# jskvrna/MonoSOWA

Hardware: AMD Instinct MI355X
Metric: MonoDETR training img/s (KITTI 1280x384) (higher is better)
Workload: dtype f32; 1 GPU; MonoDETR resnet50 KITTI 1280x384, fwd+criterion+bwd+AdamW step, per-GPU batch 16, synthetic images + random pseudo-labels; global_batch=16, per_gpu_batch=16, parallelism=dp1, accumulation_micro_steps=1, mixed_cameras=False, queries=550, tuned=True

## Files before the change

include/monosowa_attn.h:

```cpp
#ifndef MONOSOWA_ATTN_H
#define MONOSOWA_ATTN_H
#ifdef __cplusplus
extern "C" {
#endif

#define MONO_ATTN_E_NULLPTR (-1)
#define MONO_ATTN_E_SHAPE (-2)

typedef struct { long long batch, head, token; } mono_attn_strides;

int mono_attn_forward_f32(const float *q, const float *k, const float *v, float *o, float *lse, int B, int H, int Lq,
                          int Lk, int head_dim, mono_attn_strides sq, mono_attn_strides sk, mono_attn_strides sv,
                          mono_attn_strides so, float softmax_scale, float dropout_p, unsigned long long seed,
                          void *stream);

int mono_attn_backward_f32(const float *q, const float *k, const float *v, const float *o, const float *lse,
                           const float *dout, float *dq, float *dk, float *dv, float *delta, int B, int H, int Lq,
                           int Lk, int head_dim, mono_attn_strides sq, mono_attn_strides sk, mono_attn_strides sv,
                           mono_attn_strides so, mono_attn_strides sdq, mono_attn_strides sdk, mono_attn_strides sdv,
                           float softmax_scale, float dropout_p, unsigned long long seed, void *stream);

int mono_attn_forward_masked_f32(const float *q, const float *k, const float *v, const unsigned char *key_padding_mask, float *o,
                                 float *lse, int B, int H, int Lq, int Lk, int head_dim, mono_attn_strides sq,
                                 mono_attn_strides sk, mono_attn_strides sv, mono_attn_strides so, float softmax_scale,
                                 float dropout_p, unsigned long long seed, void *stream);
int mono_attn_backward_masked_f32(const float *q, const float *k, const float *v, const unsigned char *key_padding_mask,
                                  const float *o, const float *lse, const float *dout, float *dq, float *dk, float *dv, float *delta,
                                  int B, int H, int Lq, int Lk, int head_dim, mono_attn_strides sq, mono_attn_strides sk,
                                  mono_attn_strides sv, mono_attn_strides so, mono_attn_strides sdq, mono_attn_strides sdk,
                                  mono_attn_strides sdv, float softmax_scale, float dropout_p, unsigned long long seed,
                                  void *stream);

long long mono_attn_keep_words(int B, int H, int Lq, int Lk);
int mono_attn_forward_keep_f32(const float *q, const float *k, const float *v, const unsigned char *key_padding_mask,
                               unsigned *keep_bits, float *o, float *lse, int B, int H, int Lq, int Lk, int head_dim,
                               mono_attn_strides sq, mono_attn_strides sk, mono_attn_strides sv, mono_attn_strides so,
                               float softmax_scale, float dropout_p, unsigned long long seed, void *stream);
int mono_attn_backward_keep_f32(const float *q, const float *k, const float *v, const unsigned char *key_padding_mask,
                                const unsigned *keep_bits, const float *o, const float *lse, const float *dout, float *dq, float *dk,
                                float *dv, float *delta, int B, int H, int Lq, int Lk, int head_dim, mono_attn_strides sq,
                                mono_attn_strides sk, mono_attn_strides sv, mono_attn_strides so, mono_attn_strides sdq,
                                mono_attn_strides sdk, mono_attn_strides sdv, float softmax_scale, float dropout_p,
                                unsigned long long seed, void *stream);

#ifdef __cplusplus
}
#endif
#endif
```

monosowa_amd/csrc/flash_attn.hip:

```cpp
#include <hip/hip_runtime.h>

#include "../../include/monosowa_attn.h"

namespace attn {

typedef float f32x16 __attribute__((ext_vector_type(16)));

#ifndef ATTN_FWD_WAVES
#define ATTN_FWD_WAVES 4
#endif
#ifndef ATTN_BWD_WAVES
#define ATTN_BWD_WAVES 3
#endif
#ifndef ATTN_PREFETCH
#define ATTN_PREFETCH 0
#endif
#ifndef ATTN_OPDEPTH
#define ATTN_OPDEPTH 0
#endif
#ifndef ATTN_OPDEPTH_KV
#define ATTN_OPDEPTH_KV 0
#endif
#ifndef ATTN_EARLY_STORE
#define ATTN_EARLY_STORE 0
#endif
#ifndef ATTN_PRIO
#define ATTN_PRIO 0
#endif
#define ATTN_PRIO_MFMA()  do { if (ATTN_PRIO == 1) __builtin_amdgcn_s_setprio(2); else if (ATTN_PRIO == 2) __builtin_amdgcn_s_setprio(0); } while (0)
#define ATTN_PRIO_VALU()  do { if (ATTN_PRIO == 1) __builtin_amdgcn_s_setprio(0); else if (ATTN_PRIO == 2) __builtin_amdgcn_s_setprio(2); } while (0)
#ifndef ATTN_SKIP
#define ATTN_SKIP 0
#endif
constexpr int kBlockQ = 128;
constexpr int kTileK = 64;
constexpr int kKStride = 36;
constexpr int kVStride = 40;

struct Strides { long long b, h, t; };

struct Args {
  const float *q, *k, *v;
  float *o, *lse;
  const float *dout, *delta;
  float *dq, *dk, *dv;
  int H, Lq, Lk;
  Strides sq, sk, sv, so;
  Strides sdq, sdk, sdv;
  float scale_log2;
  float scale;
  unsigned drop_thr16;
  float drop_scale;
  unsigned seed_lo, seed_hi;
  const unsigned char *kmask;
  unsigned *keep;
};
__device__ __forceinline__ long long keep_index(const Args &a, int bh, int q_block, int k_tile, int slot) {
  const int n_qb = (a.Lq + 127) >> 7, n_kt = (a.Lk + 63) >> 6;
  return (((long long)bh * n_qb + q_block) * n_kt + k_tile) * 256 + slot;
}

__device__ __forceinline__ unsigned mix32(unsigned x) {
  x ^= x >> 16; x *= 0x85EBCA6Bu; x ^= x >> 13; x *= 0xC2B2AE35u; x ^= x >> 16;
  return x;
}
__device__ __forceinline__ unsigned drop_bits(unsigned head_seed, unsigned q, unsigned kp) {
  if (ATTN_SKIP & 32) return head_seed + q * 0x9E3779B1u + kp * 0x85EBCA77u;
  return mix32(head_seed + q * 0x9E3779B1u + kp * 0x85EBCA77u);
}
__device__ __forceinline__ unsigned head_seed_of(const Args &a, unsigned bh) {
  return mix32(a.seed_lo ^ (bh * 0xC2B2AE3Du)) ^ a.seed_hi;
}
__device__ __forceinline__ float4 ld4(const float *p) { return *reinterpret_cast<const float4 *>(p); }
__device__ __forceinline__ float xhalf(float v) { return __shfl_xor(v, 32); }
__device__ __forceinline__ f32x16 mfma(float a, float b, f32x16 c) { return __builtin_amdgcn_mfma_f32_32x32x2f32(a, b, c, 0, 0, 0); }

template <bool DROP, bool MASK, bool BITS>
constexpr int fwd_waves() { return (DROP && (MASK || !BITS)) ? 3 : ATTN_FWD_WAVES; }
template <bool DROP, bool MASK = false, bool BITS = false>
__global__ __launch_bounds__(256, (fwd_waves<DROP, MASK, BITS>())) void fwd_kernel(const Args a) {
  __shared__ float Ks[2][kTileK * kKStride];
  __shared__ float Vs[2][kTileK * kVStride];
  __shared__ unsigned long long Ms[2];
  const int lane = threadIdx.x & 63, wave = threadIdx.x >> 6, r = lane & 31, h = lane >> 5;
  const int bh = blockIdx.y, b = bh / a.H, hd = bh % a.H;
  const int q = blockIdx.x * kBlockQ + wave * 32 + r;
  const int qc = min(q, a.Lq - 1);
  const float *qp = a.q + b * a.sq.b + hd * a.sq.h + (long long)qc * a.sq.t + 16 * h;
  float qreg[16];
#pragma unroll
  for (int i = 0; i < 4; ++i) {
    const float4 t = ld4(qp + 4 * i);
    qreg[4 * i] = t.x * a.scale_log2; qreg[4 * i + 1] = t.y * a.scale_log2;
    qreg[4 * i + 2] = t.z * a.scale_log2; qreg[4 * i + 3] = t.w * a.scale_log2;
  }
  const float *kb = a.k + b * a.sk.b + hd * a.sk.h, *vb = a.v + b * a.sv.b + hd * a.sv.h;
  const int n_tiles = (a.Lk + kTileK - 1) / kTileK;
  float4 kr[2], vr[2];
  unsigned long long pad_next = 0;
  auto load_tile = [&](int kt) {
#pragma unroll
    for (int j = 0; j < 2; ++j) {
      const int idx = threadIdx.x + 256 * j, key = kt * kTileK + (idx >> 3), c = (idx & 7) * 4;
      const bool ok = key < a.Lk;
      kr[j] = ok ? ld4(kb + (long long)key * a.sk.t + c) : make_float4(0.f, 0.f, 0.f, 0.f);
      vr[j] = ok ? ld4(vb + (long long)key * a.sv.t + c) : make_float4(0.f, 0.f, 0.f, 0.f);
    }
    if (MASK && wave == 0) {
      const int key = kt * kTileK + lane;
      pad_next = __ballot(!(key < a.Lk && a.kmask[(long long)b * a.Lk + key] == 0));
    }
  };
  auto store_tile = [&](int buf) {
#pragma unroll
    for (int j = 0; j < 2; ++j) {
      const int idx = threadIdx.x + 256 * j, row = idx >> 3, c = (idx & 7) * 4;
      *reinterpret_cast<float4 *>(&Ks[buf][row * kKStride + c]) = kr[j];
      *reinterpret_cast<float4 *>(&Vs[buf][row * kVStride + c]) = vr[j];
    }
    if (MASK && threadIdx.x == 0) Ms[buf] = pad_next;
  };
  load_tile(0);
  store_tile(0);
  __syncthreads();

  const unsigned hseed = DROP ? head_seed_of(a, (unsigned)bh) : 0u;
  f32x16 o = {0.f, 0.f, 0.f, 0.f, 0.f, 0.f, 0.f, 0.f, 0.f, 0.f, 0.f, 0.f, 0.f, 0.f, 0.f, 0.f};
  float m = -INFINITY, lsum = 0.f;
  for (int kt = 0; kt < n_tiles; ++kt) {
    const int buf = kt & 1;
    if (kt + 1 < n_tiles) load_tile(kt + 1);
    f32x16 s0 = {0.f, 0.f, 0.f, 0.f, 0.f, 0.f, 0.f, 0.f, 0.f, 0.f, 0.f, 0.f, 0.f, 0.f, 0.f, 0.f}, s1 = s0;
    const float *k0 = &Ks[buf][r * kKStride + 16 * h], *k1 = k0 + 32 * kKStride;
    ATTN_PRIO_MFMA();
#pragma unroll
    for (int i = 0; i < 4; ++i) {
      const float4 a0 = ld4(k0 + 4 * i), a1 = ld4(k1 + 4 * i);
      s0 = mfma(a0.x, qreg[4 * i], s0);     s1 = mfma(a1.x, qreg[4 * i], s1);
      s0 = mfma(a0.y, qreg[4 * i + 1], s0); s1 = mfma(a1.y, qreg[4 * i + 1], s1);
      s0 = mfma(a0.z, qreg[4 * i + 2], s0); s1 = mfma(a1.z, qreg[4 * i + 2], s1);
      s0 = mfma(a0.w, qreg[4 * i + 3], s0); s1 = mfma(a1.w, qreg[4 * i + 3], s1);
    }
    ATTN_PRIO_VALU();
    const int key0 = kt * kTileK + 4 * h;
    if (MASK) {
      const unsigned long long tm = Ms[buf];
      const unsigned lo = __builtin_amdgcn_readfirstlane((unsigned)tm), hi = __builtin_amdgcn_readfirstlane((unsigned)(tm >> 32));
      const unsigned w0 = lo >> (4 * h), w1 = hi >> (4 * h);
#pragma unroll
      for (int v = 0; v < 16; ++v) {
        const int bit = 8 * (v >> 2) + (v & 3);
        if ((w0 >> bit) & 1u) s0[v] = -INFINITY;
        if ((w1 >> bit) & 1u) s1[v] = -INFINITY;
      }
    } else if (kt == n_tiles - 1 && (a.Lk & (kTileK - 1))) {
#pragma unroll
      for (int v = 0; v < 16; ++v) {
        const int key = key0 + 8 * (v >> 2) + (v & 3);
// ... 155 lines not shown
      for (int i = 0; i < 4; ++i) {
#if ATTN_PREFETCH
        const float4 ka = ka4[i], va = va4[i];
#else
        const float4 ka = (ATTN_SKIP & 16) ? make_float4(qreg[0], qreg[1], qreg[2], qreg[3]) : ld4(k0 + 4 * i);
        const float4 va = (ATTN_SKIP & 16) ? make_float4(doreg[0], doreg[1], doreg[2], doreg[3]) : ld4(v0 + 4 * i);
#endif
        if (ATTN_SKIP & 8) { s[i] += ka.x + ka.y + ka.z + ka.w; dp[i] += va.x + va.y + va.z + va.w; continue; }
        s = mfma(ka.x, qreg[4 * i], s);     dp = mfma(va.x, doreg[4 * i], dp);
        s = mfma(ka.y, qreg[4 * i + 1], s); dp = mfma(va.y, doreg[4 * i + 1], dp);
        s = mfma(ka.z, qreg[4 * i + 2], s); dp = mfma(va.z, doreg[4 * i + 2], dp);
        s = mfma(ka.w, qreg[4 * i + 3], s); dp = mfma(va.w, doreg[4 * i + 3], dp);
      }
      ATTN_PRIO_VALU();
      const int key0 = kt * kTileK + half * 32 + 4 * h;
      if (MASK) {
#pragma unroll
        for (int g = 0; g < 4; ++g) {
          const float4 b4 = ld4(&Bs[buf][half * 32 + 4 * h + 8 * g]);
          s[4 * g] += b4.x; s[4 * g + 1] += b4.y; s[4 * g + 2] += b4.z; s[4 * g + 3] += b4.w;
        }
      }
#pragma unroll
      for (int v = 0; v < 16; ++v) {
        const int key = key0 + 8 * (v >> 2) + (v & 3);
        float p = (ATTN_SKIP & 1) ? s[v] - lse : __builtin_amdgcn_exp2f(s[v] - lse);
        if (!MASK && key >= a.Lk) p = 0.f;
        float dpe = dp[v];
        if (DROP && !(ATTN_SKIP & 2)) {
          bool keep;
          if (saved_bits) keep = (word & (1u << (16 * half + v))) != 0;
          else {
            const unsigned bits = drop_bits(hseed, (unsigned)q, (unsigned)key >> 1);
            keep = ((key & 1) ? (bits >> 16) : (bits & 0xFFFFu)) >= a.drop_thr16;
          }
          dpe = keep ? dpe * a.drop_scale : 0.f;
        }
        s[v] = p * (dpe - delta);
      }
#if ATTN_EARLY_STORE
      if (half == 1 && kt + 1 < n_tiles) store_tile(buf ^ 1);
#endif
      ATTN_PRIO_MFMA();
#if ATTN_OPDEPTH > 0 && !ATTN_PREFETCH
      float kop[ATTN_OPDEPTH];
#pragma unroll
      for (int j = 0; j < ATTN_OPDEPTH; ++j) kop[j] = kc[(8 * (j >> 2) + (j & 3)) * kKStride];
#pragma unroll
      for (int t = 0; t < 16; ++t) {
        const float aop = kop[t % ATTN_OPDEPTH];
        if (t + ATTN_OPDEPTH < 16) {
          const int u = t + ATTN_OPDEPTH;
          kop[t % ATTN_OPDEPTH] = kc[(8 * (u >> 2) + (u & 3)) * kKStride];
        }
        dq = mfma(aop, s[t], dq);
        __builtin_amdgcn_sched_group_barrier(0x008, 1, 0);
        __builtin_amdgcn_sched_group_barrier(0x100, 1, 0);
      }
#else
#pragma unroll
      for (int t = 0; t < 16; ++t) {
        if (ATTN_SKIP & 4) { dq[t] += s[t]; continue; }
#if ATTN_PREFETCH
        dq = mfma(kq[t], s[t], dq);
#else
        dq = mfma((ATTN_SKIP & 16) ? qreg[t] : kc[(8 * (t >> 2) + (t & 3)) * kKStride], s[t], dq);
#endif
      }
#endif
    }
#if !ATTN_EARLY_STORE
    if (kt + 1 < n_tiles) store_tile(buf ^ 1);
#endif
    __syncthreads();
  }
  if (q < a.Lq) {
    float *dst = a.dq + b * a.sdq.b + hd * a.sdq.h + (long long)q * a.sdq.t + 4 * h;
#pragma unroll
    for (int g = 0; g < 4; ++g)
      *reinterpret_cast<float4 *>(dst + 8 * g) = make_float4(dq[4 * g] * a.scale, dq[4 * g + 1] * a.scale, dq[4 * g + 2] * a.scale, dq[4 * g + 3] * a.scale);
  }
}

template <bool DROP, bool MASK = false, bool BITS = false>
__global__ __launch_bounds__(256, ATTN_BWD_WAVES) void bwd_dkdv_kernel(const Args a) {
  __shared__ float Qs[2][kTileK * kKStride];
  __shared__ float Ds[2][kTileK * kKStride];
  __shared__ float Ls[2][kTileK], Es[2][kTileK];
  __shared__ unsigned Ws[2][DROP && BITS ? 256 : 4];
  const int lane = threadIdx.x & 63, wave = threadIdx.x >> 6, r = lane & 31, h = lane >> 5;
  const int bh = blockIdx.y, b = bh / a.H, hd = bh % a.H;
  const int key = blockIdx.x * kBlockQ + wave * 32 + r;
  const int wave_s = __builtin_amdgcn_readfirstlane(wave);
  const int kc_ = min(key, a.Lk - 1);
  const float *kp = a.k + b * a.sk.b + hd * a.sk.h + (long long)kc_ * a.sk.t + 16 * h;
  const float *vp = a.v + b * a.sv.b + hd * a.sv.h + (long long)kc_ * a.sv.t + 16 * h;
  float kreg[16], vreg[16];
#pragma unroll
  for (int i = 0; i < 4; ++i) {
    const float4 t = ld4(kp + 4 * i), u = ld4(vp + 4 * i);
    kreg[4 * i] = t.x * a.scale_log2; kreg[4 * i + 1] = t.y * a.scale_log2;
    kreg[4 * i + 2] = t.z * a.scale_log2; kreg[4 * i + 3] = t.w * a.scale_log2;
    vreg[4 * i] = u.x; vreg[4 * i + 1] = u.y; vreg[4 * i + 2] = u.z; vreg[4 * i + 3] = u.w;
  }
  const bool dead = MASK && a.kmask[(long long)b * a.Lk + kc_] != 0;
  const float *qb = a.q + b * a.sq.b + hd * a.sq.h, *dob = a.dout + b * a.so.b + hd * a.so.h;
  const float *lb = a.lse + (long long)bh * a.Lq, *eb = a.delta + (long long)bh * a.Lq;
  const int n_tiles = (a.Lq + kTileK - 1) / kTileK;
  float4 qr[2], dr[2];
  float lr = 0.f, er = 0.f;
  constexpr bool saved_bits = DROP && BITS;
  unsigned wr = 0;
  const int key_in_tile = (wave & 1) * 32 + r;
  const int my_half_f = (r >> 2) & 1, my_bit = 16 * (wave & 1) + 4 * (r >> 3) + (r & 3), my_ktl = wave >> 1;
  const int n_ktiles = (a.Lk + kTileK - 1) / kTileK;
  (void)key_in_tile;
  auto load_tile = [&](int qt) {
#pragma unroll
    for (int j = 0; j < 2; ++j) {
      const int idx = threadIdx.x + 256 * j, qq = qt * kTileK + (idx >> 3), c = (idx & 7) * 4;
      const bool ok = qq < a.Lq;
      qr[j] = ok ? ld4(qb + (long long)qq * a.sq.t + c) : make_float4(0.f, 0.f, 0.f, 0.f);
      dr[j] = ok ? ld4(dob + (long long)qq * a.so.t + c) : make_float4(0.f, 0.f, 0.f, 0.f);
    }
    if (threadIdx.x < kTileK) {
      const int qq = qt * kTileK + threadIdx.x;
      lr = qq < a.Lq ? lb[qq] : INFINITY;
      er = qq < a.Lq ? eb[qq] : 0.f;
    }
    if (saved_bits) {
      const int ktl = threadIdx.x >> 7, half_f = (threadIdx.x >> 6) & 1, qq = qt * kTileK + (threadIdx.x & 63);
      const int kt_f = min(2 * (int)blockIdx.x + ktl, n_ktiles - 1);
      wr = a.keep[keep_index(a, bh, qq >> 7, kt_f, ((qq & 127) >> 5) * 64 + half_f * 32 + (qq & 31))];
    }
  };
  auto store_tile = [&](int buf) {
#pragma unroll
    for (int j = 0; j < 2; ++j) {
      const int idx = threadIdx.x + 256 * j, row = idx >> 3, c = (idx & 7) * 4;
      *reinterpret_cast<float4 *>(&Qs[buf][row * kKStride + c]) = qr[j];
      *reinterpret_cast<float4 *>(&Ds[buf][row * kKStride + c]) = dr[j];
    }
    if (threadIdx.x < kTileK) { Ls[buf][threadIdx.x] = lr; Es[buf][threadIdx.x] = er; }
    if (saved_bits) Ws[buf][threadIdx.x] = wr;
  };
  load_tile(0);
  store_tile(0);
  __syncthreads();
  const unsigned hseed = DROP ? head_seed_of(a, (unsigned)bh) : 0u;
  const f32x16 zero = {0.f, 0.f, 0.f, 0.f, 0.f, 0.f, 0.f, 0.f, 0.f, 0.f, 0.f, 0.f, 0.f, 0.f, 0.f, 0.f};
  f32x16 dk = zero, dv = zero;
  for (int qt = 0; qt < n_tiles; ++qt) {
    const int buf = qt & 1;
    if (qt + 1 < n_tiles) load_tile(qt + 1);
#pragma unroll
    for (int half = 0; half < 2; ++half) {
      f32x16 s = zero, dp = zero;
      ATTN_PRIO_MFMA();
      const float *q0 = &Qs[buf][(half * 32 + r) * kKStride + 16 * h], *d0 = &Ds[buf][(half * 32 + r) * kKStride + 16 * h];
      const float *dc = &Ds[buf][(half * 32 + 4 * h) * kKStride + r], *qc = &Qs[buf][(half * 32 + 4 * h) * kKStride + r];
#if ATTN_PREFETCH
      float4 qa4[4], da4[4];
      float dcv[16], qcv[16];
#pragma unroll
      for (int i = 0; i < 4; ++i) { qa4[i] = ld4(q0 + 4 * i); da4[i] = ld4(d0 + 4 * i); }
#pragma unroll
      for (int t = 0; t < 16; ++t) {
        const int row = (8 * (t >> 2) + (t & 3)) * kKStride;
        dcv[t] = dc[row]; qcv[t] = qc[row];
      }
      __builtin_amdgcn_sched_barrier(0);
#endif
#pragma unroll
      for (int i = 0; i < 4; ++i) {
#if ATTN_PREFETCH
        const float4 qa = qa4[i], da = da4[i];
#else
        const float4 qa = (ATTN_SKIP & 16) ? make_float4(kreg[0], kreg[1], kreg[2], kreg[3]) : ld4(q0 + 4 * i);
        const float4 da = (ATTN_SKIP & 16) ? make_float4(vreg[0], vreg[1], vreg[2], vreg[3]) : ld4(d0 + 4 * i);
#endif
        if (ATTN_SKIP & 8) { s[i] += qa.x + qa.y + qa.z + qa.w; dp[i] += da.x + da.y + da.z + da.w; continue; }
        s = mfma(qa.x, kreg[4 * i], s);     dp = mfma(da.x, vreg[4 * i], dp);
        s = mfma(qa.y, kreg[4 * i + 1], s); dp = mfma(da.y, vreg[4 * i + 1], dp);
        s = mfma(qa.z, kreg[4 * i + 2], s); dp = mfma(da.z, vreg[4 * i + 2], dp);
        s = mfma(qa.w, kreg[4 * i + 3], s); dp = mfma(da.w, vreg[4 * i + 3], dp);
      }
      ATTN_PRIO_VALU();
      const int q0i = qt * kTileK + half * 32 + 4 * h;
#pragma unroll
      for (int g = 0; g < 4; ++g) {
        const float4 l4 = ld4(&Ls[buf][half * 32 + 4 * h + 8 * g]), e4 = ld4(&Es[buf][half * 32 + 4 * h + 8 * g]);
        const float ls[4] = {l4.x, l4.y, l4.z, l4.w}, es[4] = {e4.x, e4.y, e4.z, e4.w};
        uint4 w4 = make_uint4(0u, 0u, 0u, 0u);
        if (saved_bits) w4 = *reinterpret_cast<const uint4 *>(&Ws[buf][my_ktl * 128 + my_half_f * 64 + half * 32 + 4 * h + 8 * g]);
        const unsigned ws[4] = {w4.x, w4.y, w4.z, w4.w};
#pragma unroll
        for (int j = 0; j < 4; ++j) {
          const int v = 4 * g + j;
          const float p = dead ? 0.f : ((ATTN_SKIP & 1) ? s[v] - ls[j] : __builtin_amdgcn_exp2f(s[v] - ls[j]));
          float pd = p, dpe = dp[v];
          if (DROP && !(ATTN_SKIP & 2)) {
            bool keep;
            if (saved_bits) keep = ((ws[j] >> my_bit) & 1u) != 0;
            else {
              const unsigned bits = drop_bits(hseed, (unsigned)(q0i + 8 * g + j), (unsigned)key >> 1);
              keep = ((key & 1) ? (bits >> 16) : (bits & 0xFFFFu)) >= a.drop_thr16;
            }
            pd = keep ? p * a.drop_scale : 0.f;
            dpe = keep ? dpe * a.drop_scale : 0.f;
          }
          dp[v] = pd;
          s[v] = p * (dpe - es[j]);
        }
      }
      ATTN_PRIO_MFMA();
#if ATTN_EARLY_STORE
      if (half == 1 && qt + 1 < n_tiles) store_tile(buf ^ 1);
#endif
#if ATTN_OPDEPTH_KV > 0 && !ATTN_PREFETCH
      float dop[ATTN_OPDEPTH_KV], qop[ATTN_OPDEPTH_KV];
#pragma unroll
      for (int j = 0; j < ATTN_OPDEPTH_KV; ++j) {
        dop[j] = dc[(8 * (j >> 2) + (j & 3)) * kKStride];
        qop[j] = qc[(8 * (j >> 2) + (j & 3)) * kKStride];
      }
#pragma unroll
      for (int t = 0; t < 16; ++t) {
        const float da_ = dop[t % ATTN_OPDEPTH_KV], qa_ = qop[t % ATTN_OPDEPTH_KV];
        if (t + ATTN_OPDEPTH_KV < 16) {
          const int u = t + ATTN_OPDEPTH_KV, rowu = (8 * (u >> 2) + (u & 3)) * kKStride;
          dop[t % ATTN_OPDEPTH_KV] = dc[rowu];
          qop[t % ATTN_OPDEPTH_KV] = qc[rowu];
        }
        dv = mfma(da_, dp[t], dv);
        dk = mfma(qa_, s[t], dk);
      }
#else
#pragma unroll
      for (int t = 0; t < 16; ++t) {
        if (ATTN_SKIP & 4) { dv[t] += dp[t]; dk[t] += s[t]; continue; }
#if ATTN_PREFETCH
        dv = mfma(dcv[t], dp[t], dv);
        dk = mfma(qcv[t], s[t], dk);
#else
        const int row = (8 * (t >> 2) + (t & 3)) * kKStride;
        dv = mfma((ATTN_SKIP & 16) ? vreg[t] : dc[row], dp[t], dv);
        dk = mfma((ATTN_SKIP & 16) ? kreg[t] : qc[row], s[t], dk);
#endif
      }
#endif
    }
#if !ATTN_EARLY_STORE
    if (qt + 1 < n_tiles) store_tile(buf ^ 1);
#endif
    __syncthreads();
  }
  const int lane_e = (int)__builtin_amdgcn_mbcnt_hi(~0u, __builtin_amdgcn_mbcnt_lo(~0u, 0u));
  const int key_e = (int)blockIdx.x * kBlockQ + wave_s * 32 + (lane_e & 31), h_e = lane_e >> 5;
  if (key_e < a.Lk) {
    float *dkp = a.dk + b * a.sdk.b + hd * a.sdk.h + (long long)key_e * a.sdk.t + 4 * h_e;
    float *dvp = a.dv + b * a.sdv.b + hd * a.sdv.h + (long long)key_e * a.sdv.t + 4 * h_e;
#pragma unroll
    for (int g = 0; g < 4; ++g) {
      *reinterpret_cast<float4 *>(dkp + 8 * g) = make_float4(dk[4 * g] * a.scale, dk[4 * g + 1] * a.scale, dk[4 * g + 2] * a.scale, dk[4 * g + 3] * a.scale);
      *reinterpret_cast<float4 *>(dvp + 8 * g) = make_float4(dv[4 * g], dv[4 * g + 1], dv[4 * g + 2], dv[4 * g + 3]);
    }
  }
}

}

namespace {

inline attn::Strides cvt(mono_attn_strides s) { return attn::Strides{s.batch, s.head, s.token}; }

inline void fill_common(attn::Args &a, int H, int Lq, int Lk, float scale, float p, unsigned long long seed) {
  a.H = H; a.Lq = Lq; a.Lk = Lk;
  a.scale = scale;
  a.scale_log2 = scale * 1.4426950408889634f;
  a.drop_thr16 = (unsigned)(p * 65536.0f + 0.5f);
  a.drop_scale = a.drop_thr16 ? 65536.0f / (65536.0f - (float)a.drop_thr16) : 1.f;
  a.seed_lo = (unsigned)seed;
  a.seed_hi = (unsigned)(seed >> 32);
}

inline bool aligned16(const void *p, mono_attn_strides s) {
  return ((uintptr_t)p % 16 == 0) && s.batch % 4 == 0 && s.head % 4 == 0 && s.token % 4 == 0;
}

}

extern "C" {

int mono_attn_forward_f32(const float *q, const float *k, const float *v, float *o, float *lse, int B, int H, int Lq,
                          int Lk, int head_dim, mono_attn_strides sq, mono_attn_strides sk, mono_attn_strides sv,
                          mono_attn_strides so, float softmax_scale, float dropout_p, unsigned long long seed,
                          void *stream_) {
  return mono_attn_forward_masked_f32(q, k, v, nullptr, o, lse, B, H, Lq, Lk, head_dim, sq, sk, sv, so, softmax_scale, dropout_p,
                                      seed, stream_);
}

int mono_attn_forward_masked_f32(const float *q, const float *k, const float *v, const unsigned char *key_padding_mask, float *o,
                                 float *lse, int B, int H, int Lq, int Lk, int head_dim, mono_attn_strides sq,
                                 mono_attn_strides sk, mono_attn_strides sv, mono_attn_strides so, float softmax_scale,
                                 float dropout_p, unsigned long long seed, void *stream_) {
  return mono_attn_forward_keep_f32(q, k, v, key_padding_mask, nullptr, o, lse, B, H, Lq, Lk, head_dim, sq, sk, sv, so, softmax_scale,
                                    dropout_p, seed, stream_);
}

long long mono_attn_keep_words(int B, int H, int Lq, int Lk) {
  if (B <= 0 || H <= 0 || Lq <= 0 || Lk <= 0) return 0;
  return (long long)B * H * ((Lq + 127) / 128) * ((Lk + 63) / 64) * 256;
}

int mono_attn_forward_keep_f32(const float *q, const float *k, const float *v, const unsigned char *key_padding_mask,
                               unsigned *keep_bits, float *o, float *lse, int B, int H, int Lq, int Lk, int head_dim,
                               mono_attn_strides sq, mono_attn_strides sk, mono_attn_strides sv, mono_attn_strides so,
                               float softmax_scale, float dropout_p, unsigned long long seed, void *stream_) {
  if (!q || !k || !v || !o || !lse) return MONO_ATTN_E_NULLPTR;
  if (B <= 0 || H <= 0 || Lq <= 0 || Lk <= 0 || head_dim != 32 || !(dropout_p >= 0.f && dropout_p < 1.f) ||
      (long long)B * H > 65535)
    return MONO_ATTN_E_SHAPE;
  if (!aligned16(q, sq) || !aligned16(k, sk) || !aligned16(v, sv) || !aligned16(o, so)) return MONO_ATTN_E_SHAPE;
  attn::Args a{};
  a.q = q; a.k = k; a.v = v; a.o = o; a.lse = lse;
  a.sq = cvt(sq); a.sk = cvt(sk); a.sv = cvt(sv); a.so = cvt(so);
  fill_common(a, H, Lq, Lk, softmax_scale, dropout_p, seed);
  const dim3 grid((Lq + attn::kBlockQ - 1) / attn::kBlockQ, B * H);
  hipStream_t st = (hipStream_t)stream_;
  a.kmask = key_padding_mask;
  a.keep = a.drop_thr16 ? keep_bits : nullptr;
  if (key_padding_mask) {
    if (a.keep) attn::fwd_kernel<true, true, true><<<grid, 256, 0, st>>>(a);
    else if (a.drop_thr16) attn::fwd_kernel<true, true><<<grid, 256, 0, st>>>(a);
    else attn::fwd_kernel<false, true><<<grid, 256, 0, st>>>(a);
  } else if (a.keep) attn::fwd_kernel<true, false, true><<<grid, 256, 0, st>>>(a);
  else if (a.drop_thr16) attn::fwd_kernel<true><<<grid, 256, 0, st>>>(a);
  else attn::fwd_kernel<false><<<grid, 256, 0, st>>>(a);
  return (int)hipGetLastError();
}


int mono_attn_backward_f32(const float *q, const float *k, const float *v, const float *o, const float *lse,
                           const float *dout, float *dq, float *dk, float *dv, float *delta, int B, int H, int Lq,
                           int Lk, int head_dim, mono_attn_strides sq, mono_attn_strides sk, mono_attn_strides sv,
                           mono_attn_strides so, mono_attn_strides sdq, mono_attn_strides sdk, mono_attn_strides sdv,
                           float softmax_scale, float dropout_p, unsigned long long seed, void *stream_) {
  return mono_attn_backward_masked_f32(q, k, v, nullptr, o, lse, dout, dq, dk, dv, delta, B, H, Lq, Lk, head_dim, sq, sk, sv, so, sdq,
                                       sdk, sdv, softmax_scale, dropout_p, seed, stream_);
}

int mono_attn_backward_masked_f32(const float *q, const float *k, const float *v, const unsigned char *key_padding_mask,
                                  const float *o, const float *lse, const float *dout, float *dq, float *dk, float *dv, float *delta,
                                  int B, int H, int Lq, int Lk, int head_dim, mono_attn_strides sq, mono_attn_strides sk,
                                  mono_attn_strides sv, mono_attn_strides so, mono_attn_strides sdq, mono_attn_strides sdk,
                                  mono_attn_strides sdv, float softmax_scale, float dropout_p, unsigned long long seed,
                                  void *stream_) {
  return mono_attn_backward_keep_f32(q, k, v, key_padding_mask, nullptr, o, lse, dout, dq, dk, dv, delta, B, H, Lq, Lk, head_dim, sq, sk,
                                     sv, so, sdq, sdk, sdv, softmax_scale, dropout_p, seed, stream_);
}

int mono_attn_backward_keep_f32(const float *q, const float *k, const float *v, const unsigned char *key_padding_mask,
                                const unsigned *keep_bits, const float *o, const float *lse, const float *dout, float *dq, float *dk,
                                float *dv, float *delta, int B, int H, int Lq, int Lk, int head_dim, mono_attn_strides sq,
                                mono_attn_strides sk, mono_attn_strides sv, mono_attn_strides so, mono_attn_strides sdq,
                                mono_attn_strides sdk, mono_attn_strides sdv, float softmax_scale, float dropout_p,
                                unsigned long long seed, void *stream_) {
  if (!q || !k || !v || !o || !lse || !dout || !dq || !dk || !dv || !delta) return MONO_ATTN_E_NULLPTR;
  if (B <= 0 || H <= 0 || Lq <= 0 || Lk <= 0 || head_dim != 32 || !(dropout_p >= 0.f && dropout_p < 1.f) ||
      (long long)B * H > 65535)
    return MONO_ATTN_E_SHAPE;
  if (!aligned16(q, sq) || !aligned16(k, sk) || !aligned16(v, sv) || !aligned16(o, so) || !aligned16(dout, so) ||
      !aligned16(dq, sdq) || !aligned16(dk, sdk) || !aligned16(dv, sdv))
    return MONO_ATTN_E_SHAPE;
  attn::Args a{};
  a.q = q; a.k = k; a.v = v; a.o = const_cast<float *>(o); a.lse = const_cast<float *>(lse);
  a.dout = dout; a.delta = delta; a.dq = dq; a.dk = dk; a.dv = dv;
  a.sq = cvt(sq); a.sk = cvt(sk); a.sv = cvt(sv); a.so = cvt(so);
  a.sdq = cvt(sdq); a.sdk = cvt(sdk); a.sdv = cvt(sdv);
  fill_common(a, H, Lq, Lk, softmax_scale, dropout_p, seed);
  hipStream_t st = (hipStream_t)stream_;
  const dim3 gq((Lq + attn::kBlockQ - 1) / attn::kBlockQ, B * H), gk((Lk + attn::kBlockQ - 1) / attn::kBlockQ, B * H);
  a.kmask = key_padding_mask;
  a.keep = a.drop_thr16 ? const_cast<unsigned *>(keep_bits) : nullptr;
  if (key_padding_mask && a.keep) {
    attn::bwd_dq_kernel<true, true, true><<<gq, 256, 0, st>>>(a);
    attn::bwd_dkdv_kernel<true, true, true><<<gk, 256, 0, st>>>(a);
  } else if (a.keep) {
    attn::bwd_dq_kernel<true, false, true><<<gq, 256, 0, st>>>(a);
    attn::bwd_dkdv_kernel<true, false, true><<<gk, 256, 0, st>>>(a);
  } else if (key_padding_mask && a.drop_thr16) {
    attn::bwd_dq_kernel<true, true><<<gq, 256, 0, st>>>(a);
    attn::bwd_dkdv_kernel<true, true><<<gk, 256, 0, st>>>(a);
  } else if (key_padding_mask) {
    attn::bwd_dq_kernel<false, true><<<gq, 256, 0, st>>>(a);
    attn::bwd_dkdv_kernel<false, true><<<gk, 256, 0, st>>>(a);
  } else if (a.drop_thr16) {
    attn::bwd_dq_kernel<true><<<gq, 256, 0, st>>>(a);
    attn::bwd_dkdv_kernel<true><<<gk, 256, 0, st>>>(a);
  } else {
    attn::bwd_dq_kernel<false><<<gq, 256, 0, st>>>(a);
    attn::bwd_dkdv_kernel<false><<<gk, 256, 0, st>>>(a);
  }
  return (int)hipGetLastError();
}

}
```

monosowa_amd/flash_attn.py:

```python
import ctypes
import math
import os

import torch

from . import flops
from ._lib import raw_stream, on_device
from .token_linear import linear as fast_linear

_PATH = os.path.join(os.path.dirname(os.path.abspath(__file__)), "lib", "libmonosowa_attn.so")
SYMBOLS = ("mono_attn_forward_f32", "mono_attn_backward_f32", "mono_attn_forward_masked_f32", "mono_attn_backward_masked_f32",
           "mono_attn_keep_words", "mono_attn_forward_keep_f32", "mono_attn_backward_keep_f32")
_lib = None


class _Strides(ctypes.Structure):
    _fields_ = [("batch", ctypes.c_longlong), ("head", ctypes.c_longlong), ("token", ctypes.c_longlong)]


def load():
    global _lib
    if _lib is None:
        path = os.environ.get("MONOSOWA_ATTN_LIB", _PATH)
        if not os.path.exists(path):
            raise RuntimeError("HIP extension %s is missing: run `python -m monosowa_amd.build`" % path)
        lib = ctypes.CDLL(path)
        P, I, F, U = ctypes.c_void_p, ctypes.c_int, ctypes.c_float, ctypes.c_ulonglong
        lib.mono_attn_forward_f32.restype = I
        lib.mono_attn_forward_f32.argtypes = [P] * 5 + [I] * 5 + [_Strides] * 4 + [F, F, U, P]
        lib.mono_attn_backward_f32.restype = I
        lib.mono_attn_backward_f32.argtypes = [P] * 10 + [I] * 5 + [_Strides] * 7 + [F, F, U, P]
        lib.mono_attn_forward_masked_f32.restype = I
        lib.mono_attn_forward_masked_f32.argtypes = [P] * 6 + [I] * 5 + [_Strides] * 4 + [F, F, U, P]
        lib.mono_attn_backward_masked_f32.restype = I
        lib.mono_attn_backward_masked_f32.argtypes = [P] * 11 + [I] * 5 + [_Strides] * 7 + [F, F, U, P]
        lib.mono_attn_keep_words.restype = ctypes.c_longlong
        lib.mono_attn_keep_words.argtypes = [I] * 4
        lib.mono_attn_forward_keep_f32.restype = I
        lib.mono_attn_forward_keep_f32.argtypes = [P] * 7 + [I] * 5 + [_Strides] * 4 + [F, F, U, P]
        lib.mono_attn_backward_keep_f32.restype = I
        lib.mono_attn_backward_keep_f32.argtypes = [P] * 12 + [I] * 5 + [_Strides] * 7 + [F, F, U, P]
        _lib = lib
    return _lib


def _strides(t):
    assert t.stride(3) == 1
    return _Strides(t.stride(0), t.stride(1), t.stride(2))


def supported(q, k, v):
    ok = lambda t: t.is_cuda and t.dtype == torch.float32 and t.dim() == 4 and t.size(3) == 32 and t.stride(3) == 1 \
        and t.data_ptr() % 16 == 0 and all(s % 4 == 0 for s in t.stride()[:3])
    return ok(q) and ok(k) and ok(v) and q.size(0) * q.size(1) <= 65535 and k.shape == v.shape \
        and q.shape[:2] == k.shape[:2]


_seed_counter = [0]
SAVE_KEEP_BITS = os.environ.get("MONOSOWA_ATTN_KEEP_BITS", "1") != "0"


def _next_seed():
    _seed_counter[0] += 1
    rank = torch.distributed.get_rank() if torch.distributed.is_available() and torch.distributed.is_initialized() else 0
    return (torch.initial_seed() * 0x9E3779B97F4A7C15 + _seed_counter[0] * 0xD1B54A32D192ED03 + rank * 0x94D049BB133111EB) & (2 ** 63 - 1)


def _mask_ptr(mask, B, Lk):
    if mask is None:
        return 0, None
    if mask.dtype not in (torch.bool, torch.uint8) or tuple(mask.shape) != (B, Lk) or not mask.is_cuda:
        raise RuntimeError("flash_attn: key_padding_mask must be a [B, Lk] bool / uint8 tensor on the GPU (True = padding); "
                           "additive float masks take the nn.MultiheadAttention path (mha_supported)")
    if mask.dtype == torch.bool:
        mask = mask.view(torch.uint8)
    mask = mask.contiguous()
    return mask.data_ptr(), mask


def keep_bits_like(q, k, p):
    if not p > 0:
        return None
    B, H, Lq, _ = q.shape
    return torch.empty(load().mono_attn_keep_words(B, H, Lq, k.size(2)), dtype=torch.int32, device=q.device)


def forward(q, k, v, scale, p, seed, key_padding_mask=None, keep_bits=None):
    B, H, Lq, _ = q.shape
    o = torch.empty((B, H, Lq, 32), dtype=torch.float32, device=q.device)
    lse = torch.empty((B * H, Lq), dtype=torch.float32, device=q.device)
    mp, keep = _mask_ptr(key_padding_mask, B, k.size(2))
    flops.attention_forward(B, H, Lq, k.size(2))
    with on_device(q.device):
        code = load().mono_attn_forward_keep_f32(q.data_ptr(), k.data_ptr(), v.data_ptr(), mp, keep_bits.data_ptr() if keep_bits is not None else 0,
                                                 o.data_ptr(), lse.data_ptr(), B, H, Lq, k.size(2), 32, _strides(q), _strides(k), _strides(v),
                                                 _strides(o), float(scale), float(p), seed, raw_stream())
    if code:
        raise RuntimeError("mono_attn_forward_keep_f32 failed with code %d" % code)
    return o, lse


def _batch_major(t):
    return t.stride(0) >= t.stride(2)


def _like_heads(t):
    B, H, L, _ = t.shape
    if _batch_major(t):
        return torch.empty((B, L, H * 32), dtype=torch.float32, device=t.device).view(B, L, H, 32).permute(0, 2, 1, 3)
    return torch.empty((L, B, H * 32), dtype=torch.float32, device=t.device).view(L, B, H, 32).permute(1, 2, 0, 3)


def backward(q, k, v, o, lse, dout, scale, p, seed, key_padding_mask=None, keep_bits=None):
    B, H, Lq, _ = q.shape
    Lk = k.size(2)
    dq, dk, dv = _like_heads(q), _like_heads(k), _like_heads(v)
    delta = torch.empty((B * H, Lq), dtype=torch.float32, device=q.device)
    assert dout.stride() == o.stride()
    mp, keep = _mask_ptr(key_padding_mask, B, Lk)
    flops.attention_backward(B, H, Lq, Lk)
    with on_device(q.device):
        code = load().mono_attn_backward_keep_f32(q.data_ptr(), k.data_ptr(), v.data_ptr(), mp, keep_bits.data_ptr() if keep_bits is not None else 0,
                                                  o.data_ptr(), lse.data_ptr(), dout.data_ptr(), dq.data_ptr(), dk.data_ptr(), dv.data_ptr(),
                                                  delta.data_ptr(), B, H, Lq, Lk, 32, _strides(q), _strides(k), _strides(v), _strides(o),
                                                  _strides(dq), _strides(dk), _strides(dv), float(scale), float(p), seed, raw_stream())
    if code:
        raise RuntimeError("mono_attn_backward_keep_f32 failed with code %d" % code)
    return dq, dk, dv


class _Attention(torch.autograd.Function):

    @staticmethod
    def forward(ctx, q, k, v, scale, p, seed, mask=None):
        B, H, Lq, _ = q.shape
        o = _like_heads(q)
        lse = torch.empty((B * H, Lq), dtype=torch.float32, device=q.device)
        mp, mask = _mask_ptr(mask, B, k.size(2))
        bits = keep_bits_like(q, k, p) if SAVE_KEEP_BITS else None
        flops.attention_forward(B, H, Lq, k.size(2))
        with on_device(q.device):
            code = load().mono_attn_forward_keep_f32(q.data_ptr(), k.data_ptr(), v.data_ptr(), mp, bits.data_ptr() if bits is not None else 0,
                                                     o.data_ptr(), lse.data_ptr(), B, H, Lq, k.size(2), 32, _strides(q), _strides(k),
                                                     _strides(v), _strides(o), float(scale), float(p), seed, raw_stream())
        if code:
            raise RuntimeError("mono_attn_forward_keep_f32 failed with code %d" % code)
        ctx.save_for_backward(q, k, v, o, lse)
        ctx.scale, ctx.p, ctx.seed, ctx.mask, ctx.bits = scale, p, seed, mask, bits
        return o

    @staticmethod
    def backward(ctx, dout):
        q, k, v, o, lse = ctx.saved_tensors
        if dout.stride() != o.stride():
            d2 = _like_heads(o)
            d2.copy_(dout)
            dout = d2
        dq, dk, dv = backward(q, k, v, o, lse, dout, ctx.scale, ctx.p, ctx.seed, ctx.mask, ctx.bits)
        return dq, dk, dv, None, None, None, None


def attention(q, k, v, dropout_p=0.0, scale=None, seed=None, key_padding_mask=None):
    if not supported(q, k, v):
        raise RuntimeError("flash_attn.attention: unsupported tensors (need float32 GPU [B,H,L,32], 16-byte aligned strides)")
    scale = 1.0 / math.sqrt(q.size(-1)) if scale is None else scale
    if dropout_p > 0 and seed is None:
        seed = _next_seed()
    return _Attention.apply(q, k, v, scale, float(dropout_p), int(seed or 0), key_padding_mask)


def mha_forward(mha, query, key, value, key_padding_mask=None):
    E, H = mha.embed_dim, mha.num_heads
    w, bias = mha.in_proj_weight, mha.in_proj_bias
    Lq, B, _ = query.shape
    Lk = key.size(0)
    def lin2(x, w_, b_):
        if not x.is_contiguous() and x.transpose(0, 1).is_contiguous():
            a, b2 = fast_linear(x.transpose(0, 1), w_, b_).split(E, -1)
            return a.transpose(0, 1), b2.transpose(0, 1)
        return fast_linear(x, w_, b_).split(E, -1)

    def lin(x, w_, b_):
        if not x.is_contiguous() and x.transpose(0, 1).is_contiguous():
            return fast_linear(x.transpose(0, 1), w_, b_).transpose(0, 1)
        return fast_linear(x, w_, b_)
    if query is key:
        (w_qk, w_v), (b_qk, b_v) = w.split([2 * E, E]), bias.split([2 * E, E])
        q, k = lin2(query, w_qk, b_qk)
        v = lin(value, w_v, b_v)
    elif key is value:
        (w_q, w_kv), (b_q, b_kv) = w.split([E, 2 * E]), bias.split([E, 2 * E])
        q = lin(query, w_q, b_q)
        k, v = lin2(key, w_kv, b_kv)
    else:
        (w_q, w_k, w_v), (b_q, b_k, b_v) = w.split(E), bias.split(E)
        q, k, v = lin(query, w_q, b_q), lin(key, w_k, b_k), lin(value, w_v, b_v)
    heads = lambda t, L: t.unflatten(-1, (H, 32)).permute(1, 2, 0, 3)
    o = attention(heads(q, Lq), heads(k, Lk), heads(v, Lk), mha.dropout if mha.training else 0.0, key_padding_mask=key_padding_mask)
    if _batch_major(o):
        return fast_linear(o.permute(0, 2, 1, 3).reshape(B, Lq, E), mha.out_proj.weight, mha.out_proj.bias).transpose(0, 1)
    return fast_linear(o.permute(2, 0, 1, 3).reshape(Lq, B, E), mha.out_proj.weight, mha.out_proj.bias)


def mask_supported(mask, B, Lk, device):
    return mask is None or (torch.is_tensor(mask) and mask.dtype in (torch.bool, torch.uint8) and tuple(mask.shape) == (B, Lk)
                            and mask.device == device)


def mha_supported(mha, query, key, value, key_padding_mask=None):
    return (query.is_cuda and query.dtype == torch.float32 and mha.embed_dim == mha.num_heads * 32 and not mha.batch_first
# ... 4 lines not shown
```

Measured before the change: 244.6 img/s.

## Fuse attention dQ into dK/dV backward kernel with per-block partials and reduction

Adds a one-pass attention backward that computes dQ inside the dK/dV kernel. The dS tile is staged in shared memory and multiplied against K held in registers using 16x16x4 MFMA. When there are several key blocks, per-block partial dQ is written to a workspace and summed by a separate reduce kernel; a small kernel computes delta first. This removes the separate dQ kernel's recomputation of P and dS, at the cost of extra shared memory, fewer waves per SIMD (launch bound 2), an extra barrier, workspace traffic, and an allocation per call. It is on by default through an environment flag.

```diff
diff --git a/include/monosowa_attn.h b/include/monosowa_attn.h
--- a/include/monosowa_attn.h
+++ b/include/monosowa_attn.h
@@ -43,6 +43,14 @@
                                 mono_attn_strides sdk, mono_attn_strides sdv, float softmax_scale, float dropout_p,
                                 unsigned long long seed, void *stream);
 
+long long mono_attn_backward_workspace_floats(int B, int H, int Lq, int Lk);
+int mono_attn_backward_onepass_f32(const float *q, const float *k, const float *v, const unsigned char *key_padding_mask,
+                                   const unsigned *keep_bits, const float *o, const float *lse, const float *dout, float *dq, float *dk,
+                                   float *dv, float *delta, float *workspace, int B, int H, int Lq, int Lk, int head_dim,
+                                   mono_attn_strides sq, mono_attn_strides sk, mono_attn_strides sv, mono_attn_strides so,
+                                   mono_attn_strides sdq, mono_attn_strides sdk, mono_attn_strides sdv, float softmax_scale,
+                                   float dropout_p, unsigned long long seed, void *stream);
+
 #ifdef __cplusplus
 }
 #endif
diff --git a/monosowa_amd/csrc/flash_attn.hip b/monosowa_amd/csrc/flash_attn.hip
--- a/monosowa_amd/csrc/flash_attn.hip
+++ b/monosowa_amd/csrc/flash_attn.hip
@@ -5,6 +5,7 @@
 namespace attn {
 
 typedef float f32x16 __attribute__((ext_vector_type(16)));
+typedef float f32x4 __attribute__((ext_vector_type(4)));
 
 #ifndef ATTN_FWD_WAVES
 #define ATTN_FWD_WAVES 4
@@ -36,6 +37,7 @@
 constexpr int kTileK = 64;
 constexpr int kKStride = 36;
 constexpr int kVStride = 40;
+constexpr int kSStride = 136;
 
 struct Strides { long long b, h, t; };
 
@@ -54,6 +56,7 @@
   unsigned seed_lo, seed_hi;
   const unsigned char *kmask;
   unsigned *keep;
+  float *ws;
 };
 __device__ __forceinline__ long long keep_index(const Args &a, int bh, int q_block, int k_tile, int slot) {
   const int n_qb = (a.Lq + 127) >> 7, n_kt = (a.Lk + 63) >> 6;
@@ -74,6 +77,7 @@
 __device__ __forceinline__ float4 ld4(const float *p) { return *reinterpret_cast<const float4 *>(p); }
 __device__ __forceinline__ float xhalf(float v) { return __shfl_xor(v, 32); }
 __device__ __forceinline__ f32x16 mfma(float a, float b, f32x16 c) { return __builtin_amdgcn_mfma_f32_32x32x2f32(a, b, c, 0, 0, 0); }
+__device__ __forceinline__ f32x4 mfma16(float a, float b, f32x4 c) { return __builtin_amdgcn_mfma_f32_16x16x4f32(a, b, c, 0, 0, 0); }
 
 template <bool DROP, bool MASK, bool BITS>
 constexpr int fwd_waves() { return (DROP && (MASK || !BITS)) ? 3 : ATTN_FWD_WAVES; }
@@ -395,8 +399,9 @@
   }
 }
 
-template <bool DROP, bool MASK = false, bool BITS = false>
-__global__ __launch_bounds__(256, ATTN_BWD_WAVES) void bwd_dkdv_kernel(const Args a) {
+template <bool DROP, bool MASK, bool BITS, bool DQ>
+__device__ __forceinline__ void dkdv_body(const Args &a) {
+  __shared__ float Ss[DQ ? 2 : 1][DQ ? 32 * kSStride : 4];
   __shared__ float Qs[2][kTileK * kKStride];
   __shared__ float Ds[2][kTileK * kKStride];
   __shared__ float Ls[2][kTileK], Es[2][kTileK];
@@ -463,6 +468,37 @@
   const unsigned hseed = DROP ? head_seed_of(a, (unsigned)bh) : 0u;
   const f32x16 zero = {0.f, 0.f, 0.f, 0.f, 0.f, 0.f, 0.f, 0.f, 0.f, 0.f, 0.f, 0.f, 0.f, 0.f, 0.f, 0.f};
   f32x16 dk = zero, dv = zero;
+  float kq[DQ ? 32 : 1];
+  if constexpr (DQ) {
+    const float *kcol = a.k + b * a.sk.b + hd * a.sk.h + 16 * (wave_s & 1) + (lane & 15);
+#pragma unroll
+    for (int s_ = 0; s_ < 32; ++s_) {
+      const int kk = (int)blockIdx.x * kBlockQ + 16 * (s_ >> 2) + 4 * (lane >> 4) + (s_ & 3);
+      kq[s_] = kk < a.Lk ? kcol[(long long)kk * a.sk.t] : 0.f;
+    }
+  }
+  auto dq_part = [&](int qt, int half) {
+    f32x4 acc = {0.f, 0.f, 0.f, 0.f};
+    const float *sp = &Ss[half][(16 * (wave_s >> 1) + (lane & 15)) * kSStride + 4 * (lane >> 4)];
+#pragma unroll
+    for (int m = 0; m < 8; ++m) {
+      const float4 d4 = ld4(sp + 16 * m);
+      acc = mfma16(kq[4 * m], d4.x, acc);
+      acc = mfma16(kq[4 * m + 1], d4.y, acc);
+      acc = mfma16(kq[4 * m + 2], d4.z, acc);
+      acc = mfma16(kq[4 * m + 3], d4.w, acc);
+    }
+    const int qq = qt * kTileK + half * 32 + 16 * (wave_s >> 1) + (lane & 15), d0 = 16 * (wave_s & 1) + 4 * (lane >> 4);
+    if (qq < a.Lq) {
+      if (gridDim.x == 1) {
+        float *dst = a.dq + b * a.sdq.b + hd * a.sdq.h + (long long)qq * a.sdq.t + d0;
+        *reinterpret_cast<float4 *>(dst) = make_float4(acc[0] * a.scale, acc[1] * a.scale, acc[2] * a.scale, acc[3] * a.scale);
+      } else {
+        float *dst = a.ws + (((long long)blockIdx.x * gridDim.y + bh) * a.Lq + qq) * 32 + d0;
+        *reinterpret_cast<float4 *>(dst) = make_float4(acc[0], acc[1], acc[2], acc[3]);
+      }
+    }
+  };
   for (int qt = 0; qt < n_tiles; ++qt) {
     const int buf = qt & 1;
     if (qt + 1 < n_tiles) load_tile(qt + 1);
@@ -526,6 +562,12 @@
           s[v] = p * (dpe - es[j]);
         }
       }
+      if constexpr (DQ) {
+        float *sw = &Ss[half][(4 * h) * kSStride + wave * 32 + r];
+        const bool live = key < a.Lk;
+#pragma unroll
+        for (int v = 0; v < 16; ++v) sw[(8 * (v >> 2) + (v & 3)) * kSStride] = live ? s[v] : 0.f;
+      }
       ATTN_PRIO_MFMA();
 #if ATTN_EARLY_STORE
       if (half == 1 && qt + 1 < n_tiles) store_tile(buf ^ 1);
@@ -562,11 +604,18 @@
 #endif
       }
 #endif
+      if constexpr (DQ) {
+        if (half == 0) {
+          __syncthreads();
+          dq_part(qt, 0);
+        }
+      }
     }
 #if !ATTN_EARLY_STORE
     if (qt + 1 < n_tiles) store_tile(buf ^ 1);
 #endif
     __syncthreads();
+    if constexpr (DQ) dq_part(qt, 1);
   }
   const int lane_e = (int)__builtin_amdgcn_mbcnt_hi(~0u, __builtin_amdgcn_mbcnt_lo(~0u, 0u));
   const int key_e = (int)blockIdx.x * kBlockQ + wave_s * 32 + (lane_e & 31), h_e = lane_e >> 5;
@@ -579,6 +628,45 @@
       *reinterpret_cast<float4 *>(dvp + 8 * g) = make_float4(dv[4 * g], dv[4 * g + 1], dv[4 * g + 2], dv[4 * g + 3]);
     }
   }
+}
+
+template <bool DROP, bool MASK = false, bool BITS = false>
+__global__ __launch_bounds__(256, ATTN_BWD_WAVES) void bwd_dkdv_kernel(const Args a) { dkdv_body<DROP, MASK, BITS, false>(a); }
+
+template <bool DROP, bool MASK = false, bool BITS = false>
+__global__ __launch_bounds__(256, 2) void bwd_onepass_kernel(const Args a) { dkdv_body<DROP, MASK, BITS, true>(a); }
+
+__global__ __launch_bounds__(256) void bwd_delta_kernel(const Args a) {
+  const int lane = threadIdx.x & 63, wave = threadIdx.x >> 6, r = lane & 31, h = lane >> 5;
+  const int bh = blockIdx.y, b = bh / a.H, hd = bh % a.H;
+  const int q = blockIdx.x * kBlockQ + wave * 32 + r;
+  const int qc = min(q, a.Lq - 1);
+  const float *dop = a.dout + b * a.so.b + hd * a.so.h + (long long)qc * a.so.t + 16 * h;
+  const float *op = a.o + b * a.so.b + hd * a.so.h + (long long)qc * a.so.t + 16 * h;
+  float delta = 0.f;
+#pragma unroll
+  for (int i = 0; i < 4; ++i) {
+    const float4 u = ld4(dop + 4 * i), w = ld4(op + 4 * i);
+    delta += u.x * w.x + u.y * w.y + u.z * w.z + u.w * w.w;
+  }
+  delta += xhalf(delta);
+  if (h == 0 && q < a.Lq) const_cast<float *>(a.delta)[(long long)bh * a.Lq + q] = delta;
+}
+
+__global__ __launch_bounds__(256) void bwd_dq_reduce_kernel(const Args a, int n_kb) {
+  const int idx = blockIdx.x * 256 + threadIdx.x, q = idx >> 3, c = (idx & 7) * 4;
+  if (q >= a.Lq) return;
+  const int bh = blockIdx.y, b = bh / a.H, hd = bh % a.H;
+  const long long slab = (long long)gridDim.y * a.Lq * 32;
+  const float *src = a.ws + ((long long)bh * a.Lq + q) * 32 + c;
+  float4 acc = ld4(src);
+#pragma unroll 4
+  for (int kb = 1; kb < n_kb; ++kb) {
+    const float4 t = ld4(src + kb * slab);
+    acc.x += t.x; acc.y += t.y; acc.z += t.z; acc.w += t.w;
+  }
+  float *dst = a.dq + b * a.sdq.b + hd * a.sdq.h + (long long)q * a.sdq.t + c;
+  *reinterpret_cast<float4 *>(dst) = make_float4(acc.x * a.scale, acc.y * a.scale, acc.z * a.scale, acc.w * a.scale);
 }
 
 }
@@ -599,6 +687,37 @@
 
 inline bool aligned16(const void *p, mono_attn_strides s) {
   return ((uintptr_t)p % 16 == 0) && s.batch % 4 == 0 && s.head % 4 == 0 && s.token % 4 == 0;
+}
+
+int backward_args(attn::Args &a, const float *q, const float *k, const float *v, const unsigned char *key_padding_mask,
+                  const unsigned *keep_bits, const float *o, const float *lse, const float *dout, float *dq, float *dk, float *dv,
+                  float *delta, int B, int H, int Lq, int Lk, int head_dim, mono_attn_strides sq, mono_attn_strides sk,
+                  mono_attn_strides sv, mono_attn_strides so, mono_attn_strides sdq, mono_attn_strides sdk, mono_attn_strides sdv,
+                  float softmax_scale, float dropout_p, unsigned long long seed) {
+  if (!q || !k || !v || !o || !lse || !dout || !dq || !dk || !dv || !delta) return MONO_ATTN_E_NULLPTR;
+  if (B <= 0 || H <= 0 || Lq <= 0 || Lk <= 0 || head_dim != 32 || !(dropout_p >= 0.f && dropout_p < 1.f) ||
+      (long long)B * H > 65535)
+    return MONO_ATTN_E_SHAPE;
+  if (!aligned16(q, sq) || !aligned16(k, sk) || !aligned16(v, sv) || !aligned16(o, so) || !aligned16(dout, so) ||
+      !aligned16(dq, sdq) || !aligned16(dk, sdk) || !aligned16(dv, sdv))
+    return MONO_ATTN_E_SHAPE;
+  a = attn::Args{};
+  a.q = q; a.k = k; a.v = v; a.o = const_cast<float *>(o); a.lse = const_cast<float *>(lse);
+  a.dout = dout; a.delta = delta; a.dq = dq; a.dk = dk; a.dv = dv;
+  a.sq = cvt(sq); a.sk = cvt(sk); a.sv = cvt(sv); a.so = cvt(so);
+  a.sdq = cvt(sdq); a.sdk = cvt(sdk); a.sdv = cvt(sdv);
+  fill_common(a, H, Lq, Lk, softmax_scale, dropout_p, seed);
+  a.kmask = key_padding_mask;
+  a.keep = a.drop_thr16 ? const_cast<unsigned *>(keep_bits) : nullptr;
+  return 0;
+}
+
+template <bool DROP, bool MASK, bool BITS>
+void launch_onepass(const attn::Args &a, int BH, hipStream_t st) {
+  const dim3 gq((a.Lq + attn::kBlockQ - 1) / attn::kBlockQ, BH), gk((a.Lk + attn::kBlockQ - 1) / attn::kBlockQ, BH);
+  attn::bwd_delta_kernel<<<gq, 256, 0, st>>>(a);
+  attn::bwd_onepass_kernel<DROP, MASK, BITS><<<gk, 256, 0, st>>>(a);
+  if (gk.x > 1) attn::bwd_dq_reduce_kernel<<<dim3((a.Lq * 8 + 255) / 256, BH), 256, 0, st>>>(a, (int)gk.x);
 }
 
 }
@@ -679,23 +798,12 @@
                                 mono_attn_strides sk, mono_attn_strides sv, mono_attn_strides so, mono_attn_strides sdq,
                                 mono_attn_strides sdk, mono_attn_strides sdv, float softmax_scale, float dropout_p,
                                 unsigned long long seed, void *stream_) {
-  if (!q || !k || !v || !o || !lse || !dout || !dq || !dk || !dv || !delta) return MONO_ATTN_E_NULLPTR;
-  if (B <= 0 || H <= 0 || Lq <= 0 || Lk <= 0 || head_dim != 32 || !(dropout_p >= 0.f && dropout_p < 1.f) ||
-      (long long)B * H > 65535)
-    return MONO_ATTN_E_SHAPE;
-  if (!aligned16(q, sq) || !aligned16(k, sk) || !aligned16(v, sv) || !aligned16(o, so) || !aligned16(dout, so) ||
-      !aligned16(dq, sdq) || !aligned16(dk, sdk) || !aligned16(dv, sdv))
-    return MONO_ATTN_E_SHAPE;
-  attn::Args a{};
-  a.q = q; a.k = k; a.v = v; a.o = const_cast<float *>(o); a.lse = const_cast<float *>(lse);
-  a.dout = dout; a.delta = delta; a.dq = dq; a.dk = dk; a.dv = dv;
-  a.sq = cvt(sq); a.sk = cvt(sk); a.sv = cvt(sv); a.so = cvt(so);
-  a.sdq = cvt(sdq); a.sdk = cvt(sdk); a.sdv = cvt(sdv);
-  fill_common(a, H, Lq, Lk, softmax_scale, dropout_p, seed);
+  attn::Args a;
+  if (const int e = backward_args(a, q, k, v, key_padding_mask, keep_bits, o, lse, dout, dq, dk, dv, delta, B, H, Lq, Lk, head_dim, sq,
+                                  sk, sv, so, sdq, sdk, sdv, softmax_scale, dropout_p, seed))
+    return e;
   hipStream_t st = (hipStream_t)stream_;
   const dim3 gq((Lq + attn::kBlockQ - 1) / attn::kBlockQ, B * H), gk((Lk + attn::kBlockQ - 1) / attn::kBlockQ, B * H);
-  a.kmask = key_padding_mask;
-  a.keep = a.drop_thr16 ? const_cast<unsigned *>(keep_bits) : nullptr;
   if (key_padding_mask && a.keep) {
     attn::bwd_dq_kernel<true, true, true><<<gq, 256, 0, st>>>(a);
     attn::bwd_dkdv_kernel<true, true, true><<<gk, 256, 0, st>>>(a);
@@ -718,4 +826,34 @@
   return (int)hipGetLastError();
 }
 
-}
+long long mono_attn_backward_workspace_floats(int B, int H, int Lq, int Lk) {
+  if (B <= 0 || H <= 0 || Lq <= 0 || Lk <= 0) return 0;
+  const long long n_kb = (Lk + attn::kBlockQ - 1) / attn::kBlockQ;
+  return n_kb > 1 ? n_kb * B * H * Lq * 32 : 0;
+}
+
+int mono_attn_backward_onepass_f32(const float *q, const float *k, const float *v, const unsigned char *key_padding_mask,
+                                   const unsigned *keep_bits, const float *o, const float *lse, const float *dout, float *dq, float *dk,
+                                   float *dv, float *delta, float *workspace, int B, int H, int Lq, int Lk, int head_dim,
+                                   mono_attn_strides sq, mono_attn_strides sk, mono_attn_strides sv, mono_attn_strides so,
+                                   mono_attn_strides sdq, mono_attn_strides sdk, mono_attn_strides sdv, float softmax_scale,
+                                   float dropout_p, unsigned long long seed, void *stream_) {
+  attn::Args a;
+  if (const int e = backward_args(a, q, k, v, key_padding_mask, keep_bits, o, lse, dout, dq, dk, dv, delta, B, H, Lq, Lk, head_dim, sq,
+                                  sk, sv, so, sdq, sdk, sdv, softmax_scale, dropout_p, seed))
+    return e;
+  if (!workspace && mono_attn_backward_workspace_floats(B, H, Lq, Lk) > 0) return MONO_ATTN_E_NULLPTR;
+  if ((uintptr_t)workspace % 16) return MONO_ATTN_E_SHAPE;
+  a.ws = workspace;
+  hipStream_t st = (hipStream_t)stream_;
+  const int BH = B * H;
+  if (key_padding_mask && a.keep) launch_onepass<true, true, true>(a, BH, st);
+  else if (a.keep) launch_onepass<true, false, true>(a, BH, st);
+  else if (key_padding_mask && a.drop_thr16) launch_onepass<true, true, false>(a, BH, st);
+  else if (key_padding_mask) launch_onepass<false, true, false>(a, BH, st);
+  else if (a.drop_thr16) launch_onepass<true, false, false>(a, BH, st);
+  else launch_onepass<false, false, false>(a, BH, st);
+  return (int)hipGetLastError();
+}
+
+}
diff --git a/monosowa_amd/flash_attn.py b/monosowa_amd/flash_attn.py
--- a/monosowa_amd/flash_attn.py
+++ b/monosowa_amd/flash_attn.py
@@ -10,7 +10,8 @@
 
 _PATH = os.path.join(os.path.dirname(os.path.abspath(__file__)), "lib", "libmonosowa_attn.so")
 SYMBOLS = ("mono_attn_forward_f32", "mono_attn_backward_f32", "mono_attn_forward_masked_f32", "mono_attn_backward_masked_f32",
-           "mono_attn_keep_words", "mono_attn_forward_keep_f32", "mono_attn_backward_keep_f32")
+           "mono_attn_keep_words", "mono_attn_forward_keep_f32", "mono_attn_backward_keep_f32",
+           "mono_attn_backward_workspace_floats", "mono_attn_backward_onepass_f32")
 _lib = None
 
 
@@ -40,6 +41,10 @@
         lib.mono_attn_forward_keep_f32.argtypes = [P] * 7 + [I] * 5 + [_Strides] * 4 + [F, F, U, P]
         lib.mono_attn_backward_keep_f32.restype = I
         lib.mono_attn_backward_keep_f32.argtypes = [P] * 12 + [I] * 5 + [_Strides] * 7 + [F, F, U, P]
+        lib.mono_attn_backward_workspace_floats.restype = ctypes.c_longlong
+        lib.mono_attn_backward_workspace_floats.argtypes = [I] * 4
+        lib.mono_attn_backward_onepass_f32.restype = I
+        lib.mono_attn_backward_onepass_f32.argtypes = [P] * 13 + [I] * 5 + [_Strides] * 7 + [F, F, U, P]
         _lib = lib
     return _lib
 
@@ -58,6 +63,7 @@
 
 _seed_counter = [0]
 SAVE_KEEP_BITS = os.environ.get("MONOSOWA_ATTN_KEEP_BITS", "1") != "0"
+ONE_PASS_BWD = os.environ.get("MONOSOWA_ATTN_ONE_PASS", "1") != "0"
 
 
 def _next_seed():
@@ -119,13 +125,25 @@
     assert dout.stride() == o.stride()
     mp, keep = _mask_ptr(key_padding_mask, B, Lk)
     flops.attention_backward(B, H, Lq, Lk)
+    bits = keep_bits.data_ptr() if keep_bits is not None else 0
+    strides = (_strides(q), _strides(k), _strides(v), _strides(o), _strides(dq), _strides(dk), _strides(dv))
+    lib = load()
     with on_device(q.device):
-        code = load().mono_attn_backward_keep_f32(q.data_ptr(), k.data_ptr(), v.data_ptr(), mp, keep_bits.data_ptr() if keep_bits is not None else 0,
-                                                  o.data_ptr(), lse.data_ptr(), dout.data_ptr(), dq.data_ptr(), dk.data_ptr(), dv.data_ptr(),
-                                                  delta.data_ptr(), B, H, Lq, Lk, 32, _strides(q), _strides(k), _strides(v), _strides(o),
-                                                  _strides(dq), _strides(dk), _strides(dv), float(scale), float(p), seed, raw_stream())
+        if ONE_PASS_BWD:
+            name = "mono_attn_backward_onepass_f32"
+            n_ws = lib.mono_attn_backward_workspace_floats(B, H, Lq, Lk)
+            ws = torch.empty(n_ws, dtype=torch.float32, device=q.device) if n_ws else None
+            code = lib.mono_attn_backward_onepass_f32(q.data_ptr(), k.data_ptr(), v.data_ptr(), mp, bits, o.data_ptr(), lse.data_ptr(),
+                                                      dout.data_ptr(), dq.data_ptr(), dk.data_ptr(), dv.data_ptr(), delta.data_ptr(),
+                                                      ws.data_ptr() if ws is not None else 0, B, H, Lq, Lk, 32, *strides, float(scale),
+                                                      float(p), seed, raw_stream())
+        else:
+            name = "mono_attn_backward_keep_f32"
+            code = lib.mono_attn_backward_keep_f32(q.data_ptr(), k.data_ptr(), v.data_ptr(), mp, bits, o.data_ptr(), lse.data_ptr(),
+                                                   dout.data_ptr(), dq.data_ptr(), dk.data_ptr(), dv.data_ptr(), delta.data_ptr(), B, H, Lq,
+                                                   Lk, 32, *strides, float(scale), float(p), seed, raw_stream())
     if code:
-        raise RuntimeError("mono_attn_backward_keep_f32 failed with code %d" % code)
+        raise RuntimeError("%s failed with code %d" % (name, code))
     return dq, dk, dv
 
 
```

New measurement: 247.9 img/s, median of 6. 1.4% higher.
